# ustcml/RecStudio

Hardware: AMD Instinct MI355X
Metric: M scored (user,pos,neg) triplets/sec at d=128 (higher is better)
Workload: dtype f32; 1 GPU; BPR two-tower d=128, synthetic 10000001 items / 1000001 users / 1e8-interaction Zipf popularity, positives uniform over the items it holds, popular sampler neg=64, InnerProduct + BPR loss, B=65536 queries/step (BASELINE.json configs[1]); global_batch=65536, num_neg=64, dim=128, n_items=10000001, parallelism=single

## Files before the change

include/recstudio_amd.h:

```cpp
#ifndef RECSTUDIO_AMD_H
#define RECSTUDIO_AMD_H

#include <stdint.h>

#ifdef __cplusplus
extern "C" {
#endif

#define RSA_ABI_VERSION 12

typedef void* rsa_stream_t;

enum rsa_status {
  RSA_OK = 0,
  RSA_ERR_ARG = -1,
  RSA_ERR_HIP = -2,
  RSA_ERR_UNSUPPORTED = -3
};

enum rsa_score_mode { RSA_SCORE_IP = 0, RSA_SCORE_COS = 1, RSA_SCORE_EUC = 2  };
enum rsa_sampler_kind { RSA_SAMPLER_GIVEN = 0, RSA_SAMPLER_UNIFORM = 1, RSA_SAMPLER_POPULAR = 2 };
enum rsa_loss_kind { RSA_LOSS_BPR = 0, RSA_LOSS_SSM = 1, RSA_LOSS_BCE = 2,
                      RSA_LOSS_WBPR = 3, RSA_LOSS_WBCE = 4, RSA_LOSS_HINGE = 5, RSA_LOSS_NCE = 6,
                     RSA_LOSS_CCL = 7 };
// ... 100 lines not shown
  int32_t loss_kind;
  int32_t n_pos;
  const float* pos_score;
  const float* neg_score;
  const float* pos_logp;
  const float* neg_logp;
  int64_t n_rows;
  int32_t num_neg;
  int32_t _pad;
  float param0, param1;
  float* row_loss;
  float* loss_out;
  float* dpos;
  float* dneg;
  void* scratch;
} rsa_loss_args;
int rsa_pairwise_loss(const rsa_loss_args* args, rsa_stream_t stream);

int rsa_ssm_shared_loss(const rsa_loss_args* args, rsa_stream_t stream);

int rsa_mean_rows(const float* row_loss, int64_t n_rows, float* out, void* scratch, rsa_stream_t stream);

int rsa_row_lse(const float* x, int64_t n_rows, int64_t n_cols, float* lse, float* softmax_scaled,
                float scale, rsa_stream_t stream);

typedef struct rsa_backward_args {
  const float* item_table;
  int64_t n_items;
  int32_t dim;
  int32_t num_neg;
  const float* query;
  const int64_t* query_index;
  int64_t n_query_rows;
  const int64_t* pos_ids;
  const int64_t* neg_ids;
  int64_t n_queries;
  const float* dpos;
  const float* dneg;
  const float* upstream;
  float* item_grad;
  float* item_grad_rows;
  float* query_grad;
  float* query_table_grad;
  int32_t query_table_pad_row;
  int32_t item_pad_row;
  int32_t score_mode;
  int32_t _pad;
} rsa_backward_args;

int rsa_fused_backward(const rsa_backward_args* args, rsa_stream_t stream);

int64_t rsa_scatter_rows_sorted_workspace_bytes(int64_t n_queries, int32_t num_neg, int64_t n_items);

typedef struct rsa_rows_update_args {
  int64_t size;
  const float* query;
  const int64_t* query_index;
  int64_t n_query_rows;
  int32_t dim;
  int32_t has_pos;
  const int64_t* pos_ids;
  const int64_t* neg_ids;
  int64_t n_queries;
  int32_t num_neg;
  int32_t _pad;
  const float* dpos;
  const float* dneg;
  const float* upstream;
  int64_t n_items;
  int64_t pad_row;
  float* target;
  float* exp_avg;
  float* exp_avg_sq;
  double lr, beta1, beta2, eps;
  int64_t step;
  uint8_t* solo;
  void* workspace;
  int64_t workspace_bytes;
} rsa_rows_update_args;

int rsa_rows_update_sorted(const rsa_rows_update_args* args, rsa_stream_t stream);

int rsa_sort_step_elements(const rsa_rows_update_args* args, rsa_stream_t stream);
int rsa_rows_update_presorted(const rsa_rows_update_args* args, rsa_stream_t stream);

typedef struct rsa_bpr_sgd_args {
  int64_t size;
  float* item_table;
  int64_t n_items;
  float* user_table;
  int64_t n_users;
  int32_t dim;
  int32_t num_neg;
  const int64_t* user_ids;
  const int64_t* pos_ids;
  int64_t n_queries;
  int32_t sampler;
  int32_t _pad;
  const rsa_popular_args* pop;
  uint64_t seed, offset;
  uint32_t grid_threads;
  uint32_t _pad2;
  uint64_t elem_base;
  const float* step_scale;
  int64_t* neg_ids;
  uint8_t* solo;
// ... 252 lines not shown
```

recstudio_amd/_native.py:

```python
import ctypes
import os
import subprocess
from ctypes import (POINTER, Structure, c_char_p, c_double, c_float, c_int, c_int32, c_int64, c_uint32, c_uint64, c_void_p)

HERE = os.path.dirname(os.path.abspath(__file__))
LIB_PATH = os.environ.get('RSA_LIB') or os.path.join(HERE, 'librecstudio_amd.so')
CSRC = os.path.join(HERE, 'csrc')

RSA_OK = 0
SCORE_IP, SCORE_COS, SCORE_EUC = 0, 1, 2
SAMPLER_GIVEN, SAMPLER_UNIFORM, SAMPLER_POPULAR = 0, 1, 2
LOSS_BPR, LOSS_SSM, LOSS_BCE = 0, 1, 2
LOSS_WBPR, LOSS_WBCE, LOSS_HINGE, LOSS_NCE, LOSS_CCL = 3, 4, 5, 6, 7


class NativeError(RuntimeError):
    """A C-ABI call returned a negative status."""


class FusedArgs(Structure):
    _fields_ = [
        ('item_table', c_void_p), ('n_items', c_int64), ('dim', c_int32), ('score_mode', c_int32),
        ('query', c_void_p), ('query_index', c_void_p), ('n_query_rows', c_int64),
        ('pos_ids', c_void_p), ('n_queries', c_int64),
# ... 119 lines not shown
class SegGatherArgs(_Sized):
    _fields_ = [
        ('size', c_int64), ('item_table', c_void_p), ('n_items', c_int64), ('dim', c_int32), ('max_len', c_int32),
        ('flat_item_ids', c_void_p), ('n_flat', c_int64), ('seg_start', c_void_p), ('seg_end', c_void_p), ('n_seg', c_int64),
        ('out_ids', c_void_p), ('out_rows', c_void_p), ('out_len', c_void_p),
    ]


class FullscoreArgs(_Sized):
    _fields_ = [
        ('size', c_int64), ('item_table', c_void_p), ('n_items', c_int64), ('dim', c_int32), ('score_mode', c_int32),
        ('query', c_void_p), ('n_query', c_int64), ('scores', c_void_p), ('lse', c_void_p), ('topk_val', c_void_p),
        ('topk_idx', c_void_p), ('k', c_int32), ('_pad', c_int32), ('item_aux', c_void_p), ('query_aux', c_void_p),
        ('workspace', c_void_p), ('workspace_bytes', c_int64),
    ]


STRUCTS = {
    'rsa_fused_args': FusedArgs, 'rsa_backward_args': BackwardArgs, 'rsa_shard_route_args': ShardRouteArgs,
    'rsa_shard_home_args': ShardHomeArgs, 'rsa_shard_backward_args': ShardBackwardArgs,
    'rsa_shard_owner_bpr_args': ShardOwnerBprArgs, 'rsa_popular_args': PopularArgs, 'rsa_loss_args': LossArgs,
    'rsa_rows_update_args': RowsUpdateArgs, 'rsa_bpr_sgd_args': BprSgdArgs, 'rsa_seg_gather_args': SegGatherArgs,
    'rsa_fullscore_args': FullscoreArgs,
}

SIGNATURES = {
    'rsa_last_error': (c_char_p, []),
    'rsa_abi_version': (c_int, []),
    'rsa_scratch_bytes': (c_int64, []),
    'rsa_device_info': (c_int, [c_int, POINTER(c_int32), POINTER(c_int32), POINTER(c_int32)]),
    'rsa_sample_uniform': (c_int, [c_void_p, c_int64, c_int64, c_int64, c_uint64, c_uint64, c_uint32, c_uint64, c_void_p]),
    'rsa_sample_masked_uniform': (c_int, [c_void_p, c_int64, c_int32, c_int64, c_int32, c_void_p, c_uint64, c_uint64,
                                          c_uint32, c_uint64, c_void_p]),
    'rsa_sample_popular': (c_int, [POINTER(PopularArgs), c_void_p]),
    'rsa_popular_lookup': (c_int, [POINTER(PopularArgs), c_void_p]),
    'rsa_item_logp': (c_int, [c_void_p, c_int64, c_void_p, c_int64, c_void_p, c_void_p]),
    'rsa_embedding_gather': (c_int, [c_void_p, c_int64, c_int32, c_void_p, c_int64, c_void_p, c_void_p]),
    'rsa_fused_sample_gather_score': (c_int, [POINTER(FusedArgs), c_void_p]),
    'rsa_pairwise_loss': (c_int, [POINTER(LossArgs), c_void_p]),
    'rsa_ssm_shared_loss': (c_int, [POINTER(LossArgs), c_void_p]),
    'rsa_mean_rows': (c_int, [c_void_p, c_int64, c_void_p, c_void_p, c_void_p]),
    'rsa_row_lse': (c_int, [c_void_p, c_int64, c_int64, c_void_p, c_void_p, c_float, c_void_p]),
    'rsa_fused_backward': (c_int, [POINTER(BackwardArgs), c_void_p]),
    'rsa_sort_step_elements': (c_int, [POINTER(RowsUpdateArgs), c_void_p]),
    'rsa_rows_update_presorted': (c_int, [POINTER(RowsUpdateArgs), c_void_p]),
    'rsa_scatter_add_rows': (c_int, [c_void_p, c_void_p, c_int64, c_int32, c_void_p, c_int64, c_void_p]),
    'rsa_seg_gather': (c_int, [POINTER(SegGatherArgs), c_void_p]),
    'rsa_fullscore_softmax': (c_int, [c_void_p, c_int64, c_int32, c_void_p, c_int64, c_void_p, c_void_p, c_void_p,
                                      c_void_p]),
    'rsa_fullscore_softmax_dq_workspace_bytes': (c_int64, [c_int64, c_int64, c_int32]),
    'rsa_fullscore_softmax_dq': (c_int, [c_void_p, c_int64, c_int32, c_void_p, c_int64, c_void_p, c_void_p, c_void_p,
                                         c_void_p, c_void_p, c_int64, c_void_p]),
    'rsa_scatter_rows_sorted_workspace_bytes': (c_int64, [c_int64, c_int32, c_int64]),
    'rsa_rows_update_sorted': (c_int, [POINTER(RowsUpdateArgs), c_void_p]),
    'rsa_bpr_sgd_prepare': (c_int, [POINTER(BprSgdArgs), c_void_p]),
    'rsa_bpr_sgd_apply': (c_int, [POINTER(BprSgdArgs), c_void_p]),
    'rsa_probs_t_query': (c_int, [c_void_p, c_int64, c_int64, c_int64, c_void_p, c_int32, c_void_p, c_void_p]),
    'rsa_fullscore_lse_grad_workspace_bytes': (c_int64, [c_int64, c_int64, c_int32]),
    'rsa_fullscore_lse_grad': (c_int, [c_void_p, c_int64, c_int32, c_void_p, c_int64, c_void_p, c_void_p, c_void_p, c_int64, c_void_p]),
    'rsa_fullscore_softmax_dw': (c_int, [c_void_p, c_int64, c_int32, c_void_p, c_int64, c_void_p, c_void_p, c_void_p, c_void_p]),
    'rsa_rng_advance': (c_int, [c_void_p, c_uint64, c_void_p]),
    'rsa_placement_probe': (c_int, [c_void_p, c_int64, c_void_p, c_int64, c_uint32, c_void_p]),
    'rsa_row_topk': (c_int, [c_void_p, c_int64, c_int64, c_int32, c_void_p, c_void_p, c_void_p]),
    'rsa_topk_mask_history': (c_int, [c_void_p, c_void_p, c_int32, c_void_p, c_int32, c_int64, c_int32, c_void_p,
                                      c_void_p, c_void_p]),
    'rsa_shard_count': (c_int, [c_void_p, c_void_p, c_int64, c_int32, c_int64, c_int32, c_void_p, c_void_p]),
    'rsa_shard_route': (c_int, [c_void_p, c_void_p, c_int64, c_int32, c_int64, c_int32, c_int64, c_void_p, c_void_p,
                                c_void_p, c_void_p]),
    'rsa_shard_segment_stride': (c_int64, [c_int64]),
    'rsa_shard_sample_route': (c_int, [POINTER(ShardRouteArgs), c_void_p]),
    'rsa_shard_route_workgroups': (c_int64, [POINTER(ShardRouteArgs)]),
    'rsa_shard_route_query_groups': (c_int32, [c_int32, c_uint32, c_uint64, c_int32, c_int32]),
    'rsa_shard_score_segments': (c_int, [c_void_p, c_int64, c_int32, c_void_p, c_int64, c_void_p, c_int64, c_int64, c_void_p,
                                         c_void_p, c_void_p, c_void_p]),
    'rsa_shard_home': (c_int, [POINTER(ShardHomeArgs), c_void_p]),
    'rsa_shard_scatter_slots': (c_int, [c_void_p, c_void_p, c_void_p, c_int64, c_int32, c_void_p, c_void_p]),
    'rsa_shard_unpack_segments': (c_int, [c_void_p, c_int64, c_int64, c_void_p, c_void_p, c_void_p, c_void_p, c_void_p,
                                          c_void_p]),
    'rsa_shard_backward_workspace_bytes': (c_int64, [c_int64, c_int64, c_int64]),
    'rsa_shard_backward_segments': (c_int, [POINTER(ShardBackwardArgs), c_void_p]),
    'rsa_shard_pos_score': (c_int, [c_void_p, c_int64, c_int32, c_void_p, c_int64, c_void_p, c_void_p, c_void_p, c_int64, c_int32,
                                    c_int32, c_void_p]),
    'rsa_shard_owner_bpr_forward': (c_int, [POINTER(ShardOwnerBprArgs), c_void_p]),
    'rsa_shard_owner_bpr_finish': (c_int, [POINTER(ShardOwnerBprArgs), c_void_p, c_void_p]),
    'rsa_shard_owner_ssm_forward': (c_int, [POINTER(ShardOwnerBprArgs), c_void_p]),
    'rsa_shard_owner_ssm_finish': (c_int, [POINTER(ShardOwnerBprArgs), c_void_p, c_void_p]),
    'rsa_shard_unpack': (c_int, [c_void_p, c_int64, c_void_p, c_void_p, c_void_p]),
    'rsa_scatter_f32': (c_int, [c_void_p, c_void_p, c_int64, c_void_p, c_void_p]),
    'rsa_gather_f32': (c_int, [c_void_p, c_void_p, c_int64, c_void_p, c_void_p]),
    'rsa_fullscore_workspace_bytes': (c_int64, [c_int64, c_int64, c_int32]),
    'rsa_fullscore': (c_int, [POINTER(FullscoreArgs), c_void_p]),
    'rsa_row_sqnorm': (c_int, [c_void_p, c_int64, c_int32, c_int32, c_void_p, c_void_p]),
}

_lib = None


def build(verbose=False):
    out = subprocess.run(['make', '-C', CSRC, '-j8'], capture_output=True, text=True)
    if verbose or out.returncode != 0:
        print(out.stdout[-4000:])
        print(out.stderr[-4000:])
    if out.returncode != 0:
        raise RuntimeError('recstudio_amd: building librecstudio_amd.so failed')
    global _lib
    _lib = None
# ... 33 lines not shown
```

recstudio_amd/csrc/rsa_owner.hip:

```cpp
#include "rsa_common.hpp"
#include "rsa_internal.hpp"
#include "rsa_radix.hpp"
#include "rsa_tile.hpp"

#ifndef RSA_OWN_BATCH
#define RSA_OWN_BATCH 4
#endif
#ifndef RSA_OWN_MIN_WAVES
#define RSA_OWN_MIN_WAVES 1
#endif
#ifndef RSA_SSM_UPDATE_WALK
#define RSA_SSM_UPDATE_WALK 1
#endif

namespace rsa {

struct OwnArgs {
  const float* item;
  float* item_rw;
  const float* q_all;
  float* qgrad_all;
  const int64_t* keys;
  const float* d;
  const uint64_t* qpairs;
// ... 590 lines not shown
  int32_t* overflow_sticky;
  float* scale_out;
  int64_t item_pad_row;
  void* workspace;
  int64_t workspace_bytes;
  int keys_grouped;
  int no_solo = 0;
};

struct OwnPrepared {
  OwnLayout W;
  SortedLayout L;
  uint64_t* row_sorted;
  const uint64_t* q_sorted;
  int64_t slots, row_total;
  bool inplace;
};

enum OwnPrep { OWN_PREP_ALL = 0, OWN_PREP_LAYOUT = 1, OWN_PREP_SORTS = 2, OWN_PREP_SCALE = 3 };

static int owner_prepare(const OwnCommon& c, OwnPrepared& P, OwnPrep mode, hipStream_t s, const char* who) {
  RSA_CHECK_ARG(c.n_segments >= 0 && c.stride > RSA_SHARD_HDR, "%s: bad sizes", who);
  P.slots = c.n_segments * c.stride;
  RSA_CHECK_ARG(c.scale_out != nullptr, "%s: scale_out is null", who);
  RSA_CHECK_ARG(P.slots < (1ll << 31) - c.n_query_rows, "%s: more than 2^31 slots", who);
  RSA_CHECK_ARG(c.item_local && (c.q_all || mode == OWN_PREP_SORTS) && (c.keys || P.slots == 0) && c.item_target, "%s: null pointer", who);
  RSA_CHECK_ARG(c.n_rows >= 1 && c.n_rows < (1ll << 31) && c.n_query_rows >= 1 && c.n_query_rows < (1ll << 31),
                "%s: table sizes out of range", who);
  if (c.dim != 64 && c.dim != 128 && c.dim != 256) {
    rsa::set_error("%s: dim=%d: built for dim in {64, 128, 256}", who, c.dim);
    return RSA_ERR_UNSUPPORTED;
  }
  const int64_t need = own_workspace_bytes(P.slots, c.n_query_rows);
  RSA_CHECK_ARG(c.workspace && c.workspace_bytes >= need, "%s: workspace too small (%lld < %lld)", who,
                (long long)c.workspace_bytes, (long long)need);
  P.W = own_layout(c.workspace, P.slots, c.n_query_rows);
  P.row_total = P.slots + (c.pos_rows ? c.n_query_rows : 0);
  P.L = sorted_layout(P.W.sorted_ws, P.slots + c.n_query_rows);
  P.inplace = c.item_target == c.item_local;
  const unsigned row_bits = radix_key_bits(c.n_rows + 1);
  P.row_sorted = radix_result(P.L.pairs_a, P.L.pairs_b, row_bits);
  const unsigned q_bits = radix_key_bits(c.n_query_rows + 1);
  P.q_sorted = c.keys_grouped ? nullptr : radix_result(P.W.qa, P.W.qb, q_bits);
  if (mode == OWN_PREP_LAYOUT) return RSA_OK;
  if (mode != OWN_PREP_SORTS) {
    hipLaunchKernelGGL(owner_scale_kernel, dim3(1), dim3(1), 0, s, c.item_scale, c.step_dropped, c.scale_out,
                       c.overflow_sticky ? c.keys : nullptr, c.n_segments, c.stride, c.overflow_sticky);
    RSA_CHECK_LAUNCH(who);
  }
  if (mode == OWN_PREP_SCALE) return RSA_OK;
  if (P.row_total == 0) return RSA_OK;
  const RdxDiv32 by_stride = rdx_make_div32((uint64_t)c.stride);
  const SrcSegments<false> by_row{c.keys, c.pos_rows, P.slots, by_stride, (uint32_t)c.n_rows};
  if (radix_sort_pairs(by_row, P.L.pairs_a, P.L.pairs_b, P.row_total, row_bits, P.L.temp, s) != hipSuccess) {
    rsa::set_error("%s: row sort failed: %s", who, hipGetErrorString(hipGetLastError()));
    return RSA_ERR_HIP;
  }
  if (P.inplace && !c.no_solo) {
    const int rc = classify_solo(P.row_sorted, P.row_total, c.item_pad_row, c.n_rows, P.W.solo, s, who);
    if (rc != RSA_OK) return rc;
  }
  if (P.slots == 0) return RSA_OK;
  if (c.keys_grouped) {
    if (hipMemsetAsync(P.W.run_start, 0, (size_t)(2 * align256o(c.n_query_rows * 4)), s) != hipSuccess) {
      rsa::set_error("%s: memset failed", who);
      return RSA_ERR_HIP;
    }
    int64_t gblocks = (P.slots + 255) / 256;
    if (gblocks > 8192) gblocks = 8192;
    hipLaunchKernelGGL(query_runs_segments_kernel, dim3((unsigned)gblocks), dim3(256), 0, s, c.keys, P.slots, by_stride,
                       (int32_t)c.n_query_rows, P.W.run_start, P.W.run_end);
    RSA_CHECK_LAUNCH(who);
    P.q_sorted = nullptr;
    return RSA_OK;
  }
  const SrcSegments<true> by_query{c.keys, nullptr, P.slots, by_stride, (uint32_t)c.n_query_rows};
  if (radix_sort_pairs(by_query, P.W.qa, P.W.qb, P.slots, q_bits, P.W.qtemp, s) != hipSuccess) {
    rsa::set_error("%s: query sort failed: %s", who, hipGetErrorString(hipGetLastError()));
    return RSA_ERR_HIP;
  }
  if (hipMemsetAsync(P.W.run_start, 0, (size_t)(2 * align256o(c.n_query_rows * 4)), s) != hipSuccess) {
    rsa::set_error("%s: memset failed", who);
    return RSA_ERR_HIP;
  }
  int64_t blocks = (P.slots + 255) / 256;
  if (blocks > 8192) blocks = 8192;
  hipLaunchKernelGGL(query_runs_kernel, dim3((unsigned)blocks), dim3(256), 0, s, P.q_sorted, P.slots, (int32_t)c.n_query_rows,
                     P.W.run_start, P.W.run_end);
  RSA_CHECK_LAUNCH(who);
  return RSA_OK;
}

static OwnArgs walk_args(const OwnCommon& c, const OwnPrepared& P, float* qgrad_all) {
  OwnArgs o = {};
  o.item = c.item_local;
  o.item_rw = P.inplace ? c.item_target : nullptr;
  o.q_all = c.q_all;
  o.qgrad_all = qgrad_all;
  o.keys = c.keys;
  o.qpairs = P.q_sorted;
  o.run_start = P.W.run_start;
  o.run_end = P.W.run_end;
  o.solo = P.inplace ? P.W.solo : nullptr;
  o.scale = c.scale_out;
  o.n_rows = c.n_rows;
  o.n_queries = (int32_t)c.n_query_rows;
  return o;
}

}

using namespace rsa;

extern "C" int64_t rsa_shard_backward_workspace_bytes(int64_t n_segments, int64_t stride, int64_t n_query_rows) {
  if (n_segments < 0 || stride <= 0 || n_query_rows <= 0) return 0;
  return own_workspace_bytes(n_segments * stride, n_query_rows);
}

extern "C" int rsa_shard_backward_segments(const rsa_shard_backward_args* a, rsa_stream_t stream) {
  RSA_CHECK_ARG(a != nullptr, "rsa_shard_backward_segments: args is null");
  hipStream_t s = (hipStream_t)stream;
  const OwnCommon c{a->item_local, a->n_rows,       a->dim,        a->q_all,       a->n_query_rows, a->keys,
                    a->n_segments, a->stride,       nullptr,       a->item_target, a->item_scale,   const_cast<int32_t*>(a->step_dropped),
                    nullptr,       a->scale_out,    a->item_pad_row, a->workspace, a->workspace_bytes, 0};
  OwnPrepared P;
  int rc = owner_prepare(c, P, OWN_PREP_ALL, s, "rsa_shard_backward_segments");
  if (rc != RSA_OK || P.slots == 0) return rc;
  RSA_CHECK_ARG(a->d_owner && a->qgrad_all, "rsa_shard_backward_segments: null pointer");
  OwnArgs o = walk_args(c, P, a->qgrad_all);
  o.d = a->d_owner;
// ... 223 lines not shown
```

recstudio_amd/csrc/rsa_radix.hpp:

```cpp
#pragma once
#include "rsa_common.hpp"
#include <type_traits>

namespace rsa {

constexpr int RDX_DIGIT_BITS = 8;
constexpr int RDX_BINS = 1 << RDX_DIGIT_BITS;
constexpr int RDX_ITEMS = 16;
constexpr int RDX_WAVE_TILE = 64 * RDX_ITEMS;
constexpr int RDX_TILE = 4 * RDX_WAVE_TILE;
constexpr int RDX_ITEMS_MAX = 17;
constexpr int RDX_ITEMS_MIN = 4;
constexpr int RDX_SLOTS = 1024;
constexpr int RDX_INLINE_SCAN_TILES = 8;

__host__ __device__ inline uint64_t rdx_pack(uint32_t key, uint32_t val) { return ((uint64_t)key << 32) | val; }
__host__ __device__ inline uint32_t rdx_key(uint64_t p) { return (uint32_t)(p >> 32); }
__host__ __device__ inline uint32_t rdx_val(uint64_t p) { return (uint32_t)p; }

struct SrcPairs {
  const uint64_t* p;
  __device__ __forceinline__ uint64_t operator()(int64_t i) const { return p[i]; }
};

// ... 289 lines not shown
        loc[r] = c0 + rank;
        if (rank == 0) wc[d] = c0 + (uint32_t)__popcll(peers);
      }
    }
    __syncthreads();
    uint32_t inc = 0, tot_d = 0;
    if (threadIdx.x < RDX_BINS) {
      const int d = threadIdx.x;
#pragma unroll
      for (int w = 0; w < RDX_SMALL_WAVES; ++w) {
        const uint32_t c = cnt[w][d];
        cnt[w][d] = tot_d;
        tot_d += c;
      }
      inc = tot_d;
#pragma unroll
      for (int o = 1; o < 64; o <<= 1) {
        const uint32_t up = __shfl_up(inc, o, 64);
        if (lane >= o) inc += up;
      }
      if (lane == 63) s_wave[wave] = inc;
    }
    __syncthreads();
    if (threadIdx.x < RDX_BINS) {
      uint32_t before = 0;
#pragma unroll
      for (int w = 0; w < 4; ++w)
        if (w < wave) before += s_wave[w];
      dbase[threadIdx.x] = before + inc - tot_d;
    }
    __syncthreads();
#pragma unroll
    for (int r = 0; r < RDX_SMALL_ROWS; ++r) {
      if (base + r * 64 + lane < total) {
        const uint32_t d = (uint32_t)(v[r] >> shift) & (RDX_BINS - 1);
        stage[dbase[d] + cnt[wave][d] + loc[r]] = v[r];
      }
    }
    __syncthreads();
#pragma unroll
    for (int r = 0; r < RDX_SMALL_ROWS; ++r) {
      const int i = base + r * 64 + lane;
      v[r] = i < total ? stage[i] : ~0ull;
    }
    __syncthreads();
  }
#pragma unroll
  for (int r = 0; r < RDX_SMALL_ROWS; ++r) {
    const int i = base + r * 64 + lane;
    if (i < total) out[i] = v[r];
  }
}

inline unsigned radix_key_bits(int64_t n_keys) {
  unsigned b = 1;
  while (b < 32 && (1ll << b) < n_keys) ++b;
  return b;
}
inline int radix_passes(unsigned bits) { return (int)((bits + RDX_DIGIT_BITS - 1) / RDX_DIGIT_BITS); }
inline int radix_items(int64_t total) {
  const int64_t round_cap = (int64_t)RDX_SLOTS * 256 * RDX_ITEMS_MAX;
  const int64_t rounds = total <= round_cap ? 1 : (total + round_cap - 1) / round_cap;
  const int64_t per = rounds * RDX_SLOTS * 256;
  const int64_t items = (total + per - 1) / per;
  return (int)(items < RDX_ITEMS_MIN ? RDX_ITEMS_MIN : items);
}
inline int64_t radix_tiles(int64_t total) {
  const int64_t tile = 256 * (int64_t)radix_items(total);
  return (total + tile - 1) / tile;
}
inline int64_t radix_tiles_upper(int64_t max_total) {
  if (max_total <= 0) return 1;
  const int64_t by_min_tile = (max_total + 256 * (int64_t)RDX_ITEMS_MIN - 1) / (256 * (int64_t)RDX_ITEMS_MIN);
  const int64_t round_cap = (int64_t)RDX_SLOTS * 256 * RDX_ITEMS_MAX;
  const int64_t by_rounds = ((max_total + round_cap - 1) / round_cap) * RDX_SLOTS;
  return by_min_tile < by_rounds ? by_min_tile : by_rounds;
}
inline int64_t radix_temp_bytes(int64_t max_total) {
  const int64_t c = RDX_BINS * radix_tiles_upper(max_total) * 4;
  return (c + 255) / 256 * 256 + RDX_BINS * 4;
}

inline uint64_t* radix_result(uint64_t* buf_a, uint64_t* buf_b, unsigned bits) { return (radix_passes(bits) & 1) ? buf_a : buf_b; }

template <class SRC0H, class SRC0>
inline hipError_t radix_sort_pairs2(const SRC0H& src0h, const SRC0& src0, uint64_t* buf_a, uint64_t* buf_b, int64_t total,
                                    unsigned bits, void* temp, hipStream_t s);

template <class SRC0>
inline hipError_t radix_sort_pairs(const SRC0& src0, uint64_t* buf_a, uint64_t* buf_b, int64_t total, unsigned bits,
                                   void* temp, hipStream_t s) {
  return radix_sort_pairs2(src0, src0, buf_a, buf_b, total, bits, temp, s);
}

template <class SRC0H, class SRC0>
inline hipError_t radix_sort_pairs2(const SRC0H& src0h, const SRC0& src0, uint64_t* buf_a, uint64_t* buf_b, int64_t total,
                                    unsigned bits, void* temp, hipStream_t s) {
  if (total <= 0) return hipSuccess;
  if (total <= RDX_TILE) {
    if constexpr (!std::is_same<SRC0H, SRC0>::value) return hipErrorInvalidValue;
    hipLaunchKernelGGL((radix_small_kernel<SRC0>), dim3(1), dim3(64 * RDX_SMALL_WAVES), 0, s, src0, (int)total, radix_passes(bits),
                       radix_result(buf_a, buf_b, bits));
    return hipGetLastError();
  }
  const int64_t n_tiles = radix_tiles(total);
  const int items = radix_items(total);
  if (n_tiles > radix_tiles_upper(total)) return hipErrorInvalidValue;
  uint32_t* counts = reinterpret_cast<uint32_t*>(temp);
  uint32_t* totals = reinterpret_cast<uint32_t*>(reinterpret_cast<char*>(temp) + (RDX_BINS * n_tiles * 4 + 255) / 256 * 256);
  const int passes = radix_passes(bits);
  const dim3 grid((unsigned)n_tiles), block(256);
  const bool inline_scan = n_tiles <= RDX_INLINE_SCAN_TILES;
  const uint32_t* tot = inline_scan ? nullptr : totals;
  for (int p = 0; p < passes; ++p) {
    const int shift = 32 + p * RDX_DIGIT_BITS;
    uint64_t* dst = (p & 1) ? buf_b : buf_a;
    if (p == 0) {
      hipLaunchKernelGGL((radix_hist_kernel<SRC0H>), grid, block, 0, s, src0h, total, shift, n_tiles, items, counts);
      if (!inline_scan) hipLaunchKernelGGL(radix_scan_kernel, dim3(RDX_BINS), block, 0, s, counts, n_tiles, totals);
      hipLaunchKernelGGL((radix_scatter_kernel<SRC0>), grid, block, 0, s, src0, total, shift, n_tiles, items, counts, tot, dst);
    } else {
      const SrcPairs sp{(p & 1) ? buf_a : buf_b};
      hipLaunchKernelGGL((radix_hist_kernel<SrcPairs>), grid, block, 0, s, sp, total, shift, n_tiles, items, counts);
      if (!inline_scan) hipLaunchKernelGGL(radix_scan_kernel, dim3(RDX_BINS), block, 0, s, counts, n_tiles, totals);
      hipLaunchKernelGGL((radix_scatter_kernel<SrcPairs>), grid, block, 0, s, sp, total, shift, n_tiles, items, counts, tot, dst);
    }
  }
  return hipGetLastError();
}

}
```

recstudio_amd/csrc/rsa_sorted.hip:

```cpp
#include "rsa_common.hpp"
#include "rsa_radix.hpp"
#include "rsa_internal.hpp"
#include <cstring>

#ifndef RSA_SORTED_UNROLL
#define RSA_SORTED_UNROLL 4
#endif
#ifndef RSA_SORTED_NT
#define RSA_SORTED_NT 2
#endif

namespace rsa {

template <bool NT>
__device__ __forceinline__ float ld_row(const float* p) {
  if constexpr (NT) return __builtin_nontemporal_load(p);
  return *p;
}
template <bool NT>
__device__ __forceinline__ void st_row(float* p, float v) {
  if constexpr (NT) __builtin_nontemporal_store(v, p);
  else *p = v;
}

// ... 288 lines not shown
  if (dim != 64 && dim != 128 && dim != 256) {
    rsa::set_error("rsa_rows_update_sorted: dim=%d: built for dim in {64, 128, 256}", dim);
    return RSA_ERR_UNSUPPORTED;
  }
  const int ce = sorted_chunk_elems(total);
  const unsigned chunks = (unsigned)((total + ce - 1) / ce);
  dim3 grid((chunks + 3) / 4), block(256);
  const int32_t pad = (int32_t)(pad_row < 0 || pad_row >= (1ll << 31) ? -2 : pad_row);
  const bool nt = RSA_SORTED_NT == 1 || (RSA_SORTED_NT == 2 && (size_t)drop_key * dim * sizeof(float) > (512ull << 20));
#define RSA_SORTED_LAUNCH(NDW)                                                                                                 \
  if (nt) hipLaunchKernelGGL((sorted_apply_kernel<NDW, DEC, true>), grid, block, 0, s, pairs, total, query, dec, upstream, pad, \
                             (int32_t)drop_key, target, adam, L.lead_part, L.trail_part, L.meta, (int32_t)key_base,            \
                             (int32_t)elem_base, (int32_t)ce);                                                                   \
  else hipLaunchKernelGGL((sorted_apply_kernel<NDW, DEC, false>), grid, block, 0, s, pairs, total, query, dec, upstream, pad,   \
                          (int32_t)drop_key, target, adam, L.lead_part, L.trail_part, L.meta, (int32_t)key_base, (int32_t)elem_base, (int32_t)ce); \
  hipLaunchKernelGGL(sorted_finish_kernel<NDW>, grid, block, 0, s, (int64_t)chunks, upstream, pad, target, adam, L.lead_part,   \
                     L.trail_part, L.meta)
  switch (dim) {
    case 64: RSA_SORTED_LAUNCH(1); break;
    case 128: RSA_SORTED_LAUNCH(2); break;
    default: RSA_SORTED_LAUNCH(4); break;
  }
#undef RSA_SORTED_LAUNCH
  RSA_CHECK_LAUNCH("rsa_rows_update_sorted(apply)");
  return RSA_OK;
}

int apply_sorted_segments(const uint64_t* pairs, int64_t total, int64_t slots, const float* query, int32_t dim,
                          const int64_t* keys, const float* d, const float* upstream, int64_t n_rows, int64_t pad_row,
                          float* target, const SortedLayout& L, hipStream_t s) {
  const AdamArgs none{nullptr, nullptr, 0.f, 0.f, 0.f, 0.f};
  const DecSegments dec{keys, d, slots};
  return apply_sorted_pairs(pairs, total, query, dim, dec, upstream, n_rows, pad_row, target, none, L, s);
}

static unsigned step_all_bits(int64_t n_items, int64_t n_users) { return radix_key_bits(n_items + n_users + 2); }

int64_t step_all_workspace_bytes(int64_t n_queries, int32_t num_neg) { return sorted_workspace_bytes(n_queries * (int64_t)(num_neg + 2)); }

int sort_step_all(const int64_t* pos_ids, int64_t* neg_ids, const int64_t* user_ids, int64_t n_queries, int32_t num_neg,
                  int64_t n_items, int64_t n_users, uint8_t* solo, void* workspace, int64_t workspace_bytes, const StepDraw* draw,
                  hipStream_t s, const char* who) {
  const int64_t t_items = n_queries * (int64_t)(num_neg + 1), total = t_items + n_queries;
  RSA_CHECK_ARG(total < (1ll << 31) && n_items + n_users + 2 < (1ll << 31), "%s: more than 2^31 elements / keys", who);
  const int64_t need = step_all_workspace_bytes(n_queries, num_neg);
  RSA_CHECK_ARG(workspace && workspace_bytes >= need, "%s: item_workspace too small (%lld < %lld = "
                "rsa_scatter_rows_sorted_workspace_bytes(n_queries, num_neg + 1, n_items): the user rows are sorted with the item rows)",
                who, (long long)workspace_bytes, (long long)need);
  const SortedLayout L = sorted_layout(workspace, total);
  const unsigned bits = step_all_bits(n_items, n_users);
  const SrcStepIds it{pos_ids, neg_ids, n_items, num_neg, num_neg + 1, 1};
  const StepDraw none{nullptr, 0, 0, PhiloxCall{0, 0, 1, 0}, 0, 0, nullptr, nullptr, nullptr};
  const SrcStepAll<false> rd{it, user_ids, t_items, n_users, (uint32_t)(n_items + 1), none};
  hipError_t err;
  if (draw != nullptr && draw->kind != 0) {
    const SrcStepAll<true> dw{it, user_ids, t_items, n_users, (uint32_t)(n_items + 1), *draw};
    err = radix_sort_pairs2(dw, rd, L.pairs_a, L.pairs_b, total, bits, L.temp, s);
  } else {
    err = radix_sort_pairs(rd, L.pairs_a, L.pairs_b, total, bits, L.temp, s);
  }
  if (err != hipSuccess) {
    rsa::set_error("%s: radix sort failed: %s", who, hipGetErrorString(hipGetLastError()));
    return RSA_ERR_HIP;
  }
  return classify_solo(radix_result(L.pairs_a, L.pairs_b, bits), t_items, 0, n_items, solo, s, who);
}

int apply_step_all(bool users, const float* query, const int64_t* query_index, int32_t dim, int64_t n_queries, int32_t num_neg,
                   const float* dpos, const float* dneg, const float* upstream, int64_t n_items, int64_t n_users, float* target,
                   void* workspace, hipStream_t s) {
  const int64_t t_items = n_queries * (int64_t)(num_neg + 1), total = t_items + n_queries;
  const SortedLayout L = sorted_layout(workspace, total);
  const uint64_t* sorted = radix_result(L.pairs_a, L.pairs_b, step_all_bits(n_items, n_users));
  const AdamArgs none{nullptr, nullptr, 0.f, 0.f, 0.f, 0.f};
  if (!users) {
    const DecStep dec{query_index, dpos, dneg, (int)num_neg, 1};
    return apply_sorted_pairs(sorted, t_items, query, dim, dec, upstream, n_items, 0, target, none, L, s);
  }
  const DecStep dec{nullptr, nullptr, dneg, 1, 0};
  return apply_sorted_pairs(sorted + t_items, n_queries, query, dim, dec, upstream, n_users, 0, target, none, L, s, n_items + 1, t_items);
}

}

using namespace rsa;

extern "C" int64_t rsa_scatter_rows_sorted_workspace_bytes(int64_t n_queries, int32_t num_neg, int64_t n_items) {
  if (n_queries <= 0 || num_neg < 0 || n_items < 1) return 0;
  return sorted_workspace_bytes(n_queries * (int64_t)(num_neg + 1));
}

static uint64_t* step_sorted(const SortedLayout& L, int64_t n_items) {
  return radix_result(L.pairs_a, L.pairs_b, radix_key_bits(n_items + 1));
}

static int sort_elements_impl(const int64_t* pos_ids, const int64_t* neg_ids, int64_t n_queries, int32_t num_neg, int64_t n_items,
                              int64_t pad_row, uint8_t* solo, void* workspace, int64_t workspace_bytes, rsa_stream_t stream,
                              const char* who) {
  RSA_CHECK_ARG(n_queries >= 0 && num_neg >= 1 && n_items >= 1 && n_items < (1ll << 31), "%s: bad sizes", who);
  if (n_queries == 0) return RSA_OK;
  RSA_CHECK_ARG(neg_ids != nullptr, "%s: neg_ids is null", who);
  const int has_pos = pos_ids != nullptr ? 1 : 0;
  const int64_t total = n_queries * (int64_t)(num_neg + has_pos);
  RSA_CHECK_ARG(total < (1ll << 31), "%s: more than 2^31 elements", who);
  const int64_t need = rsa_scatter_rows_sorted_workspace_bytes(n_queries, num_neg, n_items);
  RSA_CHECK_ARG(workspace && workspace_bytes >= need, "%s: workspace too small (%lld < %lld)", who, (long long)workspace_bytes,
                (long long)need);
  hipStream_t s = (hipStream_t)stream;
  const SortedLayout L = sorted_layout(workspace, n_queries * (int64_t)(num_neg + 1));
  const SrcStepIds src{pos_ids, neg_ids, n_items, num_neg, num_neg + has_pos, has_pos};
  if (radix_sort_pairs(src, L.pairs_a, L.pairs_b, total, radix_key_bits(n_items + 1), L.temp, s) != hipSuccess) {
    rsa::set_error("%s: radix sort failed: %s", who, hipGetErrorString(hipGetLastError()));
    return RSA_ERR_HIP;
  }
  if (solo != nullptr) return classify_solo(step_sorted(L, n_items), total, pad_row, n_items, solo, s, who);
  return RSA_OK;
}

static int apply_sorted_impl(const float* query, const int64_t* query_index, int64_t n_query_rows, int32_t dim, int has_pos,
                             int64_t n_queries, int32_t num_neg, const float* dpos, const float* dneg, const float* upstream,
                             int64_t n_items, int64_t pad_row, float* target, AdamArgs adam, void* workspace,
                             int64_t workspace_bytes, rsa_stream_t stream) {
  RSA_CHECK_ARG(n_queries >= 0 && num_neg >= 1 && n_items >= 1 && n_items < (1ll << 31), "rsa_rows_update_sorted: bad sizes");
  if (n_queries == 0) return RSA_OK;
  RSA_CHECK_ARG(query && dneg && target, "rsa_rows_update_sorted: null pointer");
  RSA_CHECK_ARG(!has_pos || dpos != nullptr, "rsa_rows_update_sorted: pos_ids without dpos");
  RSA_CHECK_ARG(query_index != nullptr || n_query_rows >= n_queries, "rsa_rows_update_sorted: query has fewer rows than n_queries");
  const int64_t total = n_queries * (int64_t)(num_neg + has_pos);
  const int64_t need = rsa_scatter_rows_sorted_workspace_bytes(n_queries, num_neg, n_items);
  RSA_CHECK_ARG(workspace && workspace_bytes >= need, "rsa_rows_update_sorted: workspace too small (%lld < %lld)",
                (long long)workspace_bytes, (long long)need);
  const SortedLayout L = sorted_layout(workspace, n_queries * (int64_t)(num_neg + 1));
  const DecStep dec{query_index, dpos, dneg, (int)num_neg, has_pos};
  return apply_sorted_pairs(step_sorted(L, n_items), total, query, dim, dec, upstream, n_items, pad_row, target, adam, L,
                            (hipStream_t)stream);
}

static int scatter_sorted_impl(const float* query, const int64_t* query_index, int64_t n_query_rows, int32_t dim,
                               const int64_t* pos_ids, const int64_t* neg_ids, int64_t n_queries, int32_t num_neg,
                               const float* dpos, const float* dneg, const float* upstream, int64_t n_items,
                               int64_t pad_row, float* target, AdamArgs adam, void* workspace, int64_t workspace_bytes,
                               rsa_stream_t stream) {
  RSA_CHECK_ARG(pos_ids == nullptr || dpos != nullptr, "rsa_rows_update_sorted: pos_ids without dpos");
  if (dim != 64 && dim != 128 && dim != 256) {
    rsa::set_error("rsa_rows_update_sorted: dim=%d: built for dim in {64, 128, 256}", dim);
    return RSA_ERR_UNSUPPORTED;
  }
  int rc = sort_elements_impl(pos_ids, neg_ids, n_queries, num_neg, n_items, pad_row, nullptr, workspace, workspace_bytes, stream,
                              "rsa_rows_update_sorted");
  if (rc != RSA_OK) return rc;
  return apply_sorted_impl(query, query_index, n_query_rows, dim, pos_ids != nullptr, n_queries, num_neg, dpos, dneg, upstream,
                           n_items, pad_row, target, adam, workspace, workspace_bytes, stream);
}

static AdamArgs adam_of(const rsa_rows_update_args& a) {
  if (a.exp_avg == nullptr) return AdamArgs{nullptr, nullptr, 0.f, 0.f, 0.f, 0.f};
  const double bc1 = 1.0 - pow(a.beta1, (double)a.step), bc2 = 1.0 - pow(a.beta2, (double)a.step);
  return AdamArgs{a.exp_avg, a.exp_avg_sq, (float)(1.0 - a.beta1), (float)(1.0 - a.beta2), (float)a.eps,
                  (float)(a.lr * sqrt(bc2) / bc1)};
}

static int check_adam(const rsa_rows_update_args& a, const char* who) {
  if (a.exp_avg == nullptr && a.exp_avg_sq == nullptr) return RSA_OK;
  RSA_CHECK_ARG(a.exp_avg && a.exp_avg_sq && a.step >= 1 && a.beta1 >= 0.0 && a.beta1 < 1.0 && a.beta2 >= 0.0 && a.beta2 < 1.0,
                "%s: bad optimizer state / hyper-parameters", who);
  return RSA_OK;
}

// ... 23 lines not shown
```

Before: 10220 M triplets/s.

## Add MSD radix route with per-bucket LDS sort and fused solo classification

For mid-sized sorts, do one global MSD pass on the top digit, then sort each bucket's remaining low digits in shared memory inside one kernel per bucket. When requested, the same kernel also classifies solo rows, so the separate classify_solo pass is skipped. This is meant to replace several global LSD scatter passes and an extra classification pass with a single block-local sort. Buckets larger than the LDS capacity fall back to a slower in-block multipass path, and sorts above the size threshold keep the LSD route.

```diff
diff --git a/include/recstudio_amd.h b/include/recstudio_amd.h
--- a/include/recstudio_amd.h
+++ b/include/recstudio_amd.h
@@ -176,6 +176,8 @@
 
 int64_t rsa_scatter_rows_sorted_workspace_bytes(int64_t n_queries, int32_t num_neg, int64_t n_items);
 
+int rsa_radix_route(int64_t total, int32_t key_bits, int64_t* max_total, int32_t* bucket_cap);
+
 typedef struct rsa_rows_update_args {
   int64_t size;
   const float* query;
diff --git a/recstudio_amd/_native.py b/recstudio_amd/_native.py
--- a/recstudio_amd/_native.py
+++ b/recstudio_amd/_native.py
@@ -195,6 +195,7 @@
     'rsa_fullscore_softmax_dq': (c_int, [c_void_p, c_int64, c_int32, c_void_p, c_int64, c_void_p, c_void_p, c_void_p,
                                          c_void_p, c_void_p, c_int64, c_void_p]),
     'rsa_scatter_rows_sorted_workspace_bytes': (c_int64, [c_int64, c_int32, c_int64]),
+    'rsa_radix_route': (c_int, [c_int64, c_int32, POINTER(c_int64), POINTER(c_int32)]),
     'rsa_rows_update_sorted': (c_int, [POINTER(RowsUpdateArgs), c_void_p]),
     'rsa_bpr_sgd_prepare': (c_int, [POINTER(BprSgdArgs), c_void_p]),
     'rsa_bpr_sgd_apply': (c_int, [POINTER(BprSgdArgs), c_void_p]),
diff --git a/recstudio_amd/csrc/rsa_owner.hip b/recstudio_amd/csrc/rsa_owner.hip
--- a/recstudio_amd/csrc/rsa_owner.hip
+++ b/recstudio_amd/csrc/rsa_owner.hip
@@ -666,7 +666,7 @@
   if (P.row_total == 0) return RSA_OK;
   const RdxDiv32 by_stride = rdx_make_div32((uint64_t)c.stride);
   const SrcSegments<false> by_row{c.keys, c.pos_rows, P.slots, by_stride, (uint32_t)c.n_rows};
-  if (radix_sort_pairs(by_row, P.L.pairs_a, P.L.pairs_b, P.row_total, row_bits, P.L.temp, s) != hipSuccess) {
+  if (radix_sort_pairs(by_row, P.L.pairs_a, P.L.pairs_b, P.row_total, row_bits, P.L.temp, s, nullptr, false) != hipSuccess) {
     rsa::set_error("%s: row sort failed: %s", who, hipGetErrorString(hipGetLastError()));
     return RSA_ERR_HIP;
   }
@@ -689,7 +689,7 @@
     return RSA_OK;
   }
   const SrcSegments<true> by_query{c.keys, nullptr, P.slots, by_stride, (uint32_t)c.n_query_rows};
-  if (radix_sort_pairs(by_query, P.W.qa, P.W.qb, P.slots, q_bits, P.W.qtemp, s) != hipSuccess) {
+  if (radix_sort_pairs(by_query, P.W.qa, P.W.qb, P.slots, q_bits, P.W.qtemp, s, nullptr, false) != hipSuccess) {
     rsa::set_error("%s: query sort failed: %s", who, hipGetErrorString(hipGetLastError()));
     return RSA_ERR_HIP;
   }
diff --git a/recstudio_amd/csrc/rsa_radix.hpp b/recstudio_amd/csrc/rsa_radix.hpp
--- a/recstudio_amd/csrc/rsa_radix.hpp
+++ b/recstudio_amd/csrc/rsa_radix.hpp
@@ -365,6 +365,244 @@
   }
 }
 
+#ifndef RSA_RADIX_BUCKET_CAP
+#define RSA_RADIX_BUCKET_CAP 8192
+#endif
+#ifndef RSA_RADIX_MSD_MAX_TOTAL
+#define RSA_RADIX_MSD_MAX_TOTAL 1179648
+#endif
+constexpr int RDX_BKT_WAVES = 16;
+constexpr int RDX_BKT_THREADS = 64 * RDX_BKT_WAVES;
+constexpr int RDX_BKT_CAP = RSA_RADIX_BUCKET_CAP;
+constexpr int RDX_BKT_ROWS = RDX_BKT_CAP / RDX_BKT_THREADS;
+constexpr int64_t RDX_MSD_MAX_TOTAL = RSA_RADIX_MSD_MAX_TOTAL;
+static_assert(RDX_BKT_CAP % RDX_BKT_THREADS == 0 && RDX_BKT_ROWS >= 1 && RDX_BKT_ROWS <= 16, "RSA_RADIX_BUCKET_CAP: a multiple of 1024, at most 16384");
+
+struct RdxClassify {
+  uint8_t* solo;
+  int64_t classified_total;
+  int32_t pad_row, drop_key;
+  bool ran;
+};
+constexpr uint64_t RDX_SOLO_BIT = 0x80000000ull;
+
+template <int ROWS>
+__device__ __forceinline__ uint32_t rdx_bucket_rank(const uint64_t (&v)[ROWS], uint32_t (&loc)[ROWS], int rows, int base, int m,
+                                                    int shift, uint32_t (*cnt)[RDX_BINS]) {
+  const int lane = lane_id(), wave = threadIdx.x >> 6;
+  const uint64_t lt = (1ull << lane) - 1ull;
+#pragma unroll
+  for (int k = 0; k < RDX_BINS / 64; ++k) cnt[wave][k * 64 + lane] = 0;
+  __syncthreads();
+  volatile uint32_t* wc = cnt[wave];
+#pragma unroll
+  for (int r = 0; r < ROWS; ++r) {
+    loc[r] = 0;
+    if (r < rows) {
+      const bool valid = base + r * 64 + lane < m;
+      const uint32_t d = (uint32_t)(v[r] >> shift) & (RDX_BINS - 1);
+      uint64_t peers = __ballot(valid);
+#pragma unroll
+      for (int b = 0; b < RDX_DIGIT_BITS; ++b) {
+        const bool bit = (d >> b) & 1u;
+        const uint64_t bal = __ballot(bit);
+        peers &= bit ? bal : ~bal;
+      }
+      if (valid) {
+        const uint32_t c0 = wc[d];
+        const uint32_t rank = (uint32_t)__popcll(peers & lt);
+        loc[r] = c0 + rank;
+        if (rank == 0) wc[d] = c0 + (uint32_t)__popcll(peers);
+      }
+    }
+  }
+  __syncthreads();
+  uint32_t tot_d = 0;
+  if (threadIdx.x < RDX_BINS) {
+#pragma unroll
+    for (int w = 0; w < RDX_BKT_WAVES; ++w) {
+      const uint32_t c = cnt[w][threadIdx.x];
+      cnt[w][threadIdx.x] = tot_d;
+      tot_d += c;
+    }
+  }
+  __syncthreads();
+  return tot_d;
+}
+
+__device__ __forceinline__ uint32_t rdx_bucket_scan(uint32_t v, uint32_t* s_wave ) {
+  const int lane = lane_id(), wave = threadIdx.x >> 6;
+  uint32_t inc = v;
+#pragma unroll
+  for (int o = 1; o < 64; o <<= 1) {
+    const uint32_t up = __shfl_up(inc, o, 64);
+    if (lane >= o) inc += up;
+  }
+  if (wave < 4 && lane == 63) s_wave[wave] = inc;
+  __syncthreads();
+  uint32_t before = 0;
+#pragma unroll
+  for (int w = 0; w < 4; ++w)
+    if (w < wave) before += s_wave[w];
+  __syncthreads();
+  return before + inc - v;
+}
+
+__device__ __forceinline__ bool rdx_is_solo(uint32_t k, bool has_before, uint32_t before, bool has_after, uint32_t after,
+                                            const RdxClassify& cl) {
+  return !(has_before && k == before) && !(has_after && k == after) && (int32_t)k != cl.pad_row && (int32_t)k != cl.drop_key;
+}
+
+template <bool CLASSIFY>
+__global__ __launch_bounds__(RDX_BKT_THREADS) void radix_bucket_kernel(uint64_t* buf, uint64_t* other,
+                                                                       const uint32_t* __restrict__ counts,
+                                                                       const uint32_t* __restrict__ totals, int n_tiles,
+                                                                       int passes, const RdxClassify cl) {
+  __shared__ uint32_t cnt[RDX_BKT_WAVES][RDX_BINS];
+  __shared__ uint32_t dbase[RDX_BINS];
+  __shared__ uint32_t s_wave[4];
+  __shared__ uint32_t s_start, s_n, s_same;
+  __shared__ uint64_t stage[RDX_BKT_CAP];
+  const int lane = lane_id(), wave = threadIdx.x >> 6, tid = threadIdx.x;
+  {
+    uint32_t c = 0;
+    if (tid < RDX_BINS) {
+      if (totals != nullptr) {
+        c = totals[tid];
+      } else {
+        for (int t = 0; t < n_tiles; ++t) c += counts[(size_t)tid * n_tiles + t];
+      }
+    }
+    const uint32_t ex = rdx_bucket_scan(c, s_wave);
+    if (tid == (int)blockIdx.x) {
+      s_start = ex;
+      s_n = c;
+    }
+    __syncthreads();
+  }
+  const int64_t start = s_start;
+  const int n = (int)s_n;
+  if (n == 0) return;
+  uint64_t* mine = buf + start;
+  uint64_t v[RDX_BKT_ROWS];
+  uint32_t loc[RDX_BKT_ROWS];
+  if (n <= RDX_BKT_CAP) {
+    const int rows = (n + RDX_BKT_THREADS - 1) / RDX_BKT_THREADS;
+    const int base = wave * (64 * rows);
+#pragma unroll
+    for (int r = 0; r < RDX_BKT_ROWS; ++r) {
+      const int i = base + r * 64 + lane;
+      v[r] = (r < rows && i < n) ? mine[i] : ~0ull;
+    }
+    for (int p = 0; p < passes; ++p) {
+      const int shift = 32 + p * RDX_DIGIT_BITS;
+      const uint32_t tot_d = rdx_bucket_rank<RDX_BKT_ROWS>(v, loc, rows, base, n, shift, cnt);
+      const uint32_t first = rdx_bucket_scan(tot_d, s_wave);
+      if (tid < RDX_BINS) dbase[tid] = first;
+      __syncthreads();
+#pragma unroll
+      for (int r = 0; r < RDX_BKT_ROWS; ++r) {
+        if (r < rows && base + r * 64 + lane < n) {
+          const uint32_t d = (uint32_t)(v[r] >> shift) & (RDX_BINS - 1);
+          stage[dbase[d] + cnt[wave][d] + loc[r]] = v[r];
+        }
+      }
+      __syncthreads();
+#pragma unroll
+      for (int r = 0; r < RDX_BKT_ROWS; ++r) {
+        const int i = base + r * 64 + lane;
+        if (r < rows && i < n) v[r] = stage[i];
+      }
+    }
+    if (CLASSIFY && passes == 0) {
+#pragma unroll
+      for (int r = 0; r < RDX_BKT_ROWS; ++r) {
+        const int i = base + r * 64 + lane;
+        if (r < rows && i < n) stage[i] = v[r];
+      }
+      __syncthreads();
+    }
+#pragma unroll
+    for (int r = 0; r < RDX_BKT_ROWS; ++r) {
+      const int i = base + r * 64 + lane;
+      if (r < rows && i < n) {
+        uint64_t pr = v[r];
+        if (CLASSIFY && start + i < cl.classified_total) {
+          const bool hb = i > 0, ha = i + 1 < n && start + i + 1 < cl.classified_total;
+          const bool solo = rdx_is_solo(rdx_key(pr), hb, hb ? rdx_key(stage[i - 1]) : 0u, ha, ha ? rdx_key(stage[i + 1]) : 0u, cl);
+          cl.solo[rdx_val(pr)] = solo ? 1 : 0;
+          if (solo) pr |= RDX_SOLO_BIT;
+        }
+        mine[i] = pr;
+      }
+    }
+    return;
+  }
+  uint64_t* cur = mine;
+  uint64_t* alt = other + start;
+  for (int p = 0; p < passes; ++p) {
+    const int shift = 32 + p * RDX_DIGIT_BITS;
+    if (tid < RDX_BINS) dbase[tid] = 0;
+    if (tid == 0) s_same = 0;
+    __syncthreads();
+    for (int i = tid; i < n; i += RDX_BKT_THREADS) atomicAdd(&dbase[(uint32_t)(cur[i] >> shift) & (RDX_BINS - 1)], 1u);
+    __syncthreads();
+    const uint32_t c = tid < RDX_BINS ? dbase[tid] : 0u;
+    if (c == (uint32_t)n) s_same = 1;
+    const uint32_t first = rdx_bucket_scan(c, s_wave);
+    if (tid < RDX_BINS) dbase[tid] = first;
+    __syncthreads();
+    const bool same = s_same != 0;
+    __syncthreads();
+    if (same) continue;
+    for (int c0 = 0; c0 < n; c0 += RDX_BKT_CAP) {
+      const int m = n - c0 < RDX_BKT_CAP ? n - c0 : RDX_BKT_CAP;
+      const int base = wave * (64 * RDX_BKT_ROWS);
+#pragma unroll
+      for (int r = 0; r < RDX_BKT_ROWS; ++r) {
+        const int i = base + r * 64 + lane;
+        v[r] = i < m ? cur[c0 + i] : ~0ull;
+      }
+      const uint32_t tot_d = rdx_bucket_rank<RDX_BKT_ROWS>(v, loc, RDX_BKT_ROWS, base, m, shift, cnt);
+#pragma unroll
+      for (int r = 0; r < RDX_BKT_ROWS; ++r) {
+        if (base + r * 64 + lane < m) {
+          const uint32_t d = (uint32_t)(v[r] >> shift) & (RDX_BINS - 1);
+          alt[dbase[d] + cnt[wave][d] + loc[r]] = v[r];
+        }
+      }
+      __syncthreads();
+      if (tid < RDX_BINS) dbase[tid] += tot_d;
+    }
+    __syncthreads();
+    uint64_t* t = cur;
+    cur = alt;
+    alt = t;
+  }
+  if (cur != mine) {
+    for (int i = tid; i < n; i += RDX_BKT_THREADS) mine[i] = cur[i];
+    __syncthreads();
+  }
+  if (CLASSIFY) {
+    for (int i0 = 0; i0 < n; i0 += RDX_BKT_THREADS) {
+      const int i = i0 + tid;
+      uint64_t pr = 0;
+      bool solo = false;
+      const bool act = i < n && start + i < cl.classified_total;
+      if (act) {
+        pr = mine[i];
+        const bool hb = i > 0, ha = i + 1 < n && start + i + 1 < cl.classified_total;
+        solo = rdx_is_solo(rdx_key(pr), hb, hb ? rdx_key(mine[i - 1]) : 0u, ha, ha ? rdx_key(mine[i + 1]) : 0u, cl);
+      }
+      __syncthreads();
+      if (act) {
+        cl.solo[rdx_val(pr)] = solo ? 1 : 0;
+        if (solo) mine[i] = pr | RDX_SOLO_BIT;
+      }
+    }
+  }
+}
+
 inline unsigned radix_key_bits(int64_t n_keys) {
   unsigned b = 1;
   while (b < 32 && (1ll << b) < n_keys) ++b;
@@ -394,23 +632,35 @@
   return (c + 255) / 256 * 256 + RDX_BINS * 4;
 }
 
+constexpr int RDX_ROUTE_SMALL = 0;
+constexpr int RDX_ROUTE_MSD = 1;
+constexpr int RDX_ROUTE_LSD = 2;
+inline unsigned radix_msd_low_bits(unsigned bits) { return bits > (unsigned)RDX_DIGIT_BITS ? bits - RDX_DIGIT_BITS : 0u; }
+inline int radix_route(int64_t total, unsigned bits) {
+  (void)bits;
+  if (total <= RDX_TILE) return RDX_ROUTE_SMALL;
+  return total <= RDX_MSD_MAX_TOTAL ? RDX_ROUTE_MSD : RDX_ROUTE_LSD;
+}
+
 inline uint64_t* radix_result(uint64_t* buf_a, uint64_t* buf_b, unsigned bits) { return (radix_passes(bits) & 1) ? buf_a : buf_b; }
 
 template <class SRC0H, class SRC0>
 inline hipError_t radix_sort_pairs2(const SRC0H& src0h, const SRC0& src0, uint64_t* buf_a, uint64_t* buf_b, int64_t total,
-                                    unsigned bits, void* temp, hipStream_t s);
+                                    unsigned bits, void* temp, hipStream_t s, RdxClassify* cl = nullptr, bool allow_msd = true);
 
 template <class SRC0>
 inline hipError_t radix_sort_pairs(const SRC0& src0, uint64_t* buf_a, uint64_t* buf_b, int64_t total, unsigned bits,
-                                   void* temp, hipStream_t s) {
-  return radix_sort_pairs2(src0, src0, buf_a, buf_b, total, bits, temp, s);
+                                   void* temp, hipStream_t s, RdxClassify* cl = nullptr, bool allow_msd = true) {
+  return radix_sort_pairs2(src0, src0, buf_a, buf_b, total, bits, temp, s, cl, allow_msd);
 }
 
 template <class SRC0H, class SRC0>
 inline hipError_t radix_sort_pairs2(const SRC0H& src0h, const SRC0& src0, uint64_t* buf_a, uint64_t* buf_b, int64_t total,
-                                    unsigned bits, void* temp, hipStream_t s) {
+                                    unsigned bits, void* temp, hipStream_t s, RdxClassify* cl, bool allow_msd) {
+  if (cl) cl->ran = false;
   if (total <= 0) return hipSuccess;
-  if (total <= RDX_TILE) {
+  const int route = radix_route(total, bits);
+  if (route == RDX_ROUTE_SMALL) {
     if constexpr (!std::is_same<SRC0H, SRC0>::value) return hipErrorInvalidValue;
     hipLaunchKernelGGL((radix_small_kernel<SRC0>), dim3(1), dim3(64 * RDX_SMALL_WAVES), 0, s, src0, (int)total, radix_passes(bits),
                        radix_result(buf_a, buf_b, bits));
@@ -425,6 +675,25 @@
   const dim3 grid((unsigned)n_tiles), block(256);
   const bool inline_scan = n_tiles <= RDX_INLINE_SCAN_TILES;
   const uint32_t* tot = inline_scan ? nullptr : totals;
+  if (route == RDX_ROUTE_MSD && allow_msd) {
+    const unsigned low = radix_msd_low_bits(bits);
+    const int shift = 32 + (int)low, low_passes = radix_passes(low);
+    uint64_t* dst = radix_result(buf_a, buf_b, bits);
+    uint64_t* other = dst == buf_a ? buf_b : buf_a;
+    hipLaunchKernelGGL((radix_hist_kernel<SRC0H>), grid, block, 0, s, src0h, total, shift, n_tiles, items, counts);
+    if (!inline_scan) hipLaunchKernelGGL(radix_scan_kernel, dim3(RDX_BINS), block, 0, s, counts, n_tiles, totals);
+    hipLaunchKernelGGL((radix_scatter_kernel<SRC0>), grid, block, 0, s, src0, total, shift, n_tiles, items, counts, tot, dst);
+    if (cl != nullptr) {
+      hipLaunchKernelGGL(radix_bucket_kernel<true>, dim3(RDX_BINS), dim3(RDX_BKT_THREADS), 0, s, dst, other, counts, tot, (int)n_tiles,
+                         low_passes, *cl);
+      cl->ran = true;
+    } else if (low_passes > 0) {
+      const RdxClassify none{nullptr, 0, 0, 0, false};
+      hipLaunchKernelGGL(radix_bucket_kernel<false>, dim3(RDX_BINS), dim3(RDX_BKT_THREADS), 0, s, dst, other, counts, tot, (int)n_tiles,
+                         low_passes, none);
+    }
+    return hipGetLastError();
+  }
   for (int p = 0; p < passes; ++p) {
     const int shift = 32 + p * RDX_DIGIT_BITS;
     uint64_t* dst = (p & 1) ? buf_b : buf_a;
diff --git a/recstudio_amd/csrc/rsa_sorted.hip b/recstudio_amd/csrc/rsa_sorted.hip
--- a/recstudio_amd/csrc/rsa_sorted.hip
+++ b/recstudio_amd/csrc/rsa_sorted.hip
@@ -364,17 +364,19 @@
   const SrcStepIds it{pos_ids, neg_ids, n_items, num_neg, num_neg + 1, 1};
   const StepDraw none{nullptr, 0, 0, PhiloxCall{0, 0, 1, 0}, 0, 0, nullptr, nullptr, nullptr};
   const SrcStepAll<false> rd{it, user_ids, t_items, n_users, (uint32_t)(n_items + 1), none};
+  RdxClassify cl{solo, t_items, 0, (int32_t)n_items, false};
   hipError_t err;
   if (draw != nullptr && draw->kind != 0) {
     const SrcStepAll<true> dw{it, user_ids, t_items, n_users, (uint32_t)(n_items + 1), *draw};
-    err = radix_sort_pairs2(dw, rd, L.pairs_a, L.pairs_b, total, bits, L.temp, s);
+    err = radix_sort_pairs2(dw, rd, L.pairs_a, L.pairs_b, total, bits, L.temp, s, &cl);
   } else {
-    err = radix_sort_pairs(rd, L.pairs_a, L.pairs_b, total, bits, L.temp, s);
+    err = radix_sort_pairs(rd, L.pairs_a, L.pairs_b, total, bits, L.temp, s, &cl);
   }
   if (err != hipSuccess) {
     rsa::set_error("%s: radix sort failed: %s", who, hipGetErrorString(hipGetLastError()));
     return RSA_ERR_HIP;
   }
+  if (cl.ran) return RSA_OK;
   return classify_solo(radix_result(L.pairs_a, L.pairs_b, bits), t_items, 0, n_items, solo, s, who);
 }
 
@@ -396,6 +398,13 @@
 }
 
 using namespace rsa;
+
+extern "C" int rsa_radix_route(int64_t total, int32_t key_bits, int64_t* max_total, int32_t* bucket_cap) {
+  if (max_total) *max_total = RDX_MSD_MAX_TOTAL;
+  if (bucket_cap) *bucket_cap = RDX_BKT_CAP;
+  if (total <= 0 || key_bits < 1 || key_bits > 32) return -1;
+  return radix_route(total, (unsigned)key_bits);
+}
 
 extern "C" int64_t rsa_scatter_rows_sorted_workspace_bytes(int64_t n_queries, int32_t num_neg, int64_t n_items) {
   if (n_queries <= 0 || num_neg < 0 || n_items < 1) return 0;
@@ -421,11 +430,13 @@
   hipStream_t s = (hipStream_t)stream;
   const SortedLayout L = sorted_layout(workspace, n_queries * (int64_t)(num_neg + 1));
   const SrcStepIds src{pos_ids, neg_ids, n_items, num_neg, num_neg + has_pos, has_pos};
-  if (radix_sort_pairs(src, L.pairs_a, L.pairs_b, total, radix_key_bits(n_items + 1), L.temp, s) != hipSuccess) {
+  RdxClassify cl{solo, total, (int32_t)(pad_row < 0 || pad_row >= (1ll << 31) ? -2 : pad_row), (int32_t)n_items, false};
+  if (radix_sort_pairs(src, L.pairs_a, L.pairs_b, total, radix_key_bits(n_items + 1), L.temp, s, solo != nullptr ? &cl : nullptr) !=
+      hipSuccess) {
     rsa::set_error("%s: radix sort failed: %s", who, hipGetErrorString(hipGetLastError()));
     return RSA_ERR_HIP;
   }
-  if (solo != nullptr) return classify_solo(step_sorted(L, n_items), total, pad_row, n_items, solo, s, who);
+  if (solo != nullptr && !cl.ran) return classify_solo(step_sorted(L, n_items), total, pad_row, n_items, solo, s, who);
   return RSA_OK;
 }
 
```

Result: slower. 8780 M triplets/s (-14.1%).
